# Lumina-Group/libzkp

Hardware: NVIDIA B200
Metric: groth16_bn254_proofs_per_sec_batched (higher is better)
Workload: dtype u256 (8x32-bit Montgomery limbs, integer)

## Files before the change

### libzkp_b200/csrc/engine.cu

```cuda
#include <cuda_runtime.h>
#include <atomic>
#include <cmath>
#include <cstdio>
#include <cstdlib>
#include <mutex>
#include <string>
#include <thread>
#include <type_traits>
#include <vector>

#include "common.h"
#include "host_util.h"
#include "kernels_prove.cuh"
#include "tables.h"
#include "large.h"
#include "setup.h"
#include "verify.h"

using namespace lzkp;
using namespace lzkp::eng;

static thread_local std::string g_err;
static std::mutex g_mu;
static int g_device = -1;
static std::vector<int> g_devices;
static thread_local int t_device = -1;
static uint64_t g_mimc_uploaded = 0;
static std::atomic<int> g_profile{0};

namespace lzkp {
namespace eng {
std::atomic<uint64_t> g_launches{0};
int fail(int code, const std::string &msg) {
    g_err = msg;
    return code;
}
int DBuf::alloc(size_t n) {
    release();
    if (n == 0) n = 16;
    cudaError_t e = cudaMalloc(&p, n);
    if (e != cudaSuccess) {
        p = nullptr;
        cudaGetLastError();
        return fail(LZKP_E_NOMEM, "cudaMalloc(" + std::to_string(n) + "): " + cudaGetErrorString(e));
    }
    bytes = n;
    return LZKP_OK;
}
void DBuf::release() {
    if (p) cudaFree(p);
    p = nullptr;
    bytes = 0;
}
int ensure_device() {
    std::lock_guard<std::mutex> lk(g_mu);
    if (g_device < 0) {
        int n = 0;
        cudaError_t e = cudaGetDeviceCount(&n);
        if (e != cudaSuccess || n == 0) {
            cudaGetLastError();
            return fail(LZKP_E_NO_DEVICE, "no CUDA device: this engine has no CPU fallback");
        }
        int dev = 0;
        if (const char *lr = getenv("LOCAL_RANK")) dev = atoi(lr) % n;
        g_device = dev;
    }
    const int dev = t_device >= 0 ? t_device : g_device;
    CUDA_TRY(cudaSetDevice(dev));
    if (!(g_mimc_uploaded >> (dev & 63) & 1)) {
        std::vector<Fr> c(110);
        for (uint32_t i = 0; i < 110; i++) c[i] = host::mimc_constant(i);
        CUDA_TRY(cudaMemcpyToSymbol(c_mimc, c.data(), sizeof(Fr) * 110));
        g_mimc_uploaded |= 1ull << (dev & 63);
    }
    return LZKP_OK;
}
int current_device() { return t_device >= 0 ? t_device : g_device; }
DeviceScope::DeviceScope(int dev) : prev(t_device) {
    t_device = dev;
    cudaSetDevice(dev);
}
DeviceScope::~DeviceScope() {
    t_device = prev;
    const int back = prev >= 0 ? prev : g_device;
    if (back >= 0) cudaSetDevice(back);
}
}
}


struct MsmPlan {
    DBuf table;
    DBuf unit_dig, unit_tbl;
    DBuf items[4];
    DBuf msm_items[4];
    uint32_t n_items[4] = {0, 0, 0, 0};
    uint32_t n_units = 0, n_rows = 0, n_msm = 0;
    std::vector<uint32_t> msm_unit_begin;
    std::vector<uint2> msm_items_host[4];
};
static const uint32_t kUnitsPerItem[4] = {8, 32, 128, 512};

struct HBuf {
    void *p = nullptr;
    size_t bytes = 0;
    int ensure(size_t n) {
        if (n <= bytes) return LZKP_OK;
        if (p) cudaFreeHost(p);
        p = nullptr;
        bytes = 0;
        cudaError_t err = cudaMallocHost(&p, n);
        if (err != cudaSuccess) { p = nullptr; cudaGetLastError(); return fail(LZKP_E_NOMEM, "cudaMallocHost failed"); }
        bytes = n;
        return LZKP_OK;
    }
    template <class T> T *as() const { return reinterpret_cast<T *>(p); }
    ~HBuf() { if (p) cudaFreeHost(p); }
};
struct Workspace {
    uint32_t chunk = 0;
    DBuf z, abc, tmp, h, dig, r, s, rs, part1, part2, res1, res2, proofs, status, a, b, commit, sets, setlen, env, envlen;
    HBuf h_proofs, h_status, h_commit, h_env, h_envlen;
    cudaEvent_t last_use = nullptr;
    ~Workspace() { if (last_use) cudaEventDestroy(last_use); }
};
static int ws_acquire(Workspace &ws, cudaStream_t st) {
    if (!ws.last_use) CUDA_TRY(cudaEventCreateWithFlags(&ws.last_use, cudaEventDisableTiming));
    else CUDA_TRY(cudaStreamWaitEvent(st, ws.last_use, 0));
    return LZKP_OK;
}
static int ws_release(Workspace &ws, cudaStream_t st) {
    CUDA_TRY(cudaEventRecord(ws.last_use, st));
    return LZKP_OK;
}

struct lzkp_pk {
    std::mutex mu;
    int device = 0;
    std::vector<lzkp_pk *> replicas;
    uint32_t n_vars = 0, n_inst = 0, n_wit = 0, n = 0, log_n = 0, m = 0;
    bool has_circuit = false;
    int kind = -1;
    uint32_t kind_param = 0;
    int c = 16;
    uint32_t W = 16, N = 32768;
    uint64_t table_bytes = 0;
    uint32_t max_chunk = 8192;
    uint32_t n_dig_rows = 0, nz = 0;
    MsmPlan g1, g2;
    MsmPlan g1_lat;
    uint32_t row_sz = 0, row_rz = 0;
    bool has_lat = false;
    ProofConsts consts;
    DBuf csr_rowptr[3], csr_col[3], csr_val[3];
    CsrDev csr[3];
    DBuf tw_fwd, tw_inv, coset_br, uncoset_br;
    NttTables ntt;
    Workspace ws[2];
    bool large = false;
    bool tiled_wm = false;
    MsmBases *L_a = nullptr, *L_b1 = nullptr, *L_b2 = nullptr, *L_l = nullptr, *L_h = nullptr;
    DBuf L_sa, L_sb, L_sl, L_sb1;
    cudaStream_t L_st[3] = {nullptr, nullptr, nullptr}, L_st_scale = nullptr;
    cudaEvent_t L_ev_in = nullptr, L_ev_done[3] = {nullptr, nullptr, nullptr}, L_ev_a = nullptr, L_ev_scale = nullptr;
    uint32_t shard_index = 0, shard_count = 1, map_ranks = 1;
    bool L_scaled = false;
    uint32_t L_lo[5] = {0, 0, 0, 0, 0}, L_cnt[5] = {0, 0, 0, 0, 0};
    cudaStream_t stream = nullptr, stream2 = nullptr;
    cudaEvent_t ev_fork = nullptr, ev_join[2] = {nullptr, nullptr};
    cudaStream_t chunk_stream(int i) const { return (i & 1) ? stream2 : stream; }
    struct Mark { int region; cudaEvent_t a, b; };
    std::vector<Mark> marks;
    double prof_ms[LZKP_PROFILE_REGIONS] = {0};
    uint64_t prof_count[LZKP_PROFILE_REGIONS] = {0};
    ~lzkp_pk() {
        for (lzkp_pk *r : replicas) { DeviceScope ds(r->device); delete r; }
        for (auto &m : marks) { cudaEventDestroy(m.a); cudaEventDestroy(m.b); }
        for (MsmBases *b : {L_a, L_b1, L_b2, L_l, L_h}) if (b) msm_bases_free(b);
        for (auto s_ : L_st) if (s_) cudaStreamDestroy(s_);
        if (L_ev_in) cudaEventDestroy(L_ev_in);
        if (L_ev_a) cudaEventDestroy(L_ev_a);
        if (L_ev_scale) cudaEventDestroy(L_ev_scale);
        if (L_st_scale) cudaStreamDestroy(L_st_scale);
        for (auto ev : L_ev_done) if (ev) cudaEventDestroy(ev);
        if (ev_fork) cudaEventDestroy(ev_fork);
        for (auto ev : ev_join) if (ev) cudaEventDestroy(ev);
        if (stream2) cudaStreamDestroy(stream2);
        if (stream) cudaStreamDestroy(stream);
    }
};

struct BaseRef { uint32_t dig_row, tbl_row; };
static int finish_plan(MsmPlan &pl, const std::vector<std::vector<BaseRef>> &msms, uint32_t W) {
    std::vector<uint32_t> ud, ut;
    pl.msm_unit_begin.clear();
    for (auto &ms : msms) {
        pl.msm_unit_begin.push_back((uint32_t)ud.size());
        for (auto &b : ms)
            for (uint32_t w = 0; w < W; w++) {
                ud.push_back(b.dig_row * W + w);
                ut.push_back(b.tbl_row * W + w);
            }
    }
    pl.msm_unit_begin.push_back((uint32_t)ud.size());
    pl.n_units = (uint32_t)ud.size();
    pl.n_msm = (uint32_t)msms.size();
    TRY(upload(pl.unit_dig, ud));
    TRY(upload(pl.unit_tbl, ut));
    for (int v = 0; v < 4; v++) {
        std::vector<uint2> items, mi;
        for (uint32_t q = 0; q < pl.n_msm; q++) {
            uint32_t first = (uint32_t)items.size();
            for (uint32_t u = pl.msm_unit_begin[q]; u < pl.msm_unit_begin[q + 1]; u += kUnitsPerItem[v])
                items.push_back(make_uint2(u, std::min(u + kUnitsPerItem[v], pl.msm_unit_begin[q + 1])));
            mi.push_back(make_uint2(first, (uint32_t)items.size()));
        }
        pl.n_items[v] = (uint32_t)items.size();
        pl.msm_items_host[v] = mi;
        TRY(upload(pl.items[v], items));
        TRY(upload(pl.msm_items[v], mi));
    }
    return LZKP_OK;
}

static inline uint32_t window_count(int c) { return (uint32_t)((255 + c - 1) / c); }

namespace {
struct Reader {
    const uint8_t *p, *end;
    bool take(size_t n, const uint8_t **out) {
        if ((size_t)(end - p) < n) return false;
        *out = p;
        p += n;
        return true;
    }
    bool g1(host::G1Canon &o) { const uint8_t *b; return take(64, &b) && host::read_g1(b, o); }
    bool g2(host::G2Canon &o) { const uint8_t *b; return take(128, &b) && host::read_g2(b, o); }
    bool vec_g1(std::vector<host::G1Canon> &v) {
        const uint8_t *b;
        if (!take(8, &b)) return false;
        uint64_t len;
        memcpy(&len, b, 8);
        if (len > (uint64_t)(end - p) / 64) return false;
        v.resize(len);
        for (auto &x : v) if (!g1(x)) return false;
        return true;
    }
    bool vec_g2(std::vector<host::G2Canon> &v) {
        const uint8_t *b;
        if (!take(8, &b)) return false;
        uint64_t len;
        memcpy(&len, b, 8);
        if (len > (uint64_t)(end - p) / 128) return false;
        v.resize(len);
        for (auto &x : v) if (!g2(x)) return false;
        return true;
    }
};
host::G1Canon neg_canon(const host::G1Canon &p) {
    host::G1Canon r = p;
    if (!host::is_inf(p)) {
        Fq m = Fq::modulus();
        sub8(r.y.l, m.l, p.y.l);
    }
    return r;
}
}

static int pk_load_impl(const uint8_t *bytes, size_t len, int validate, const lzkp_pk_options *opt, lzkp_pk *pk) {
    static_assert(sizeof(host::G1Canon) == sizeof(G1Affine) && sizeof(host::G2Canon) == sizeof(G2Affine), "layout");
    Reader rd{bytes, bytes + len};
    host::G1Canon alpha_g1, beta_g1, delta_g1;
    host::G2Canon beta_g2, gamma_g2, delta_g2;
    std::vector<host::G1Canon> gamma_abc, a_q, b1_q, h_q, l_q;
    std::vector<host::G2Canon> b2_q;
    bool ok = rd.g1(alpha_g1) && rd.g2(beta_g2) && rd.g2(gamma_g2) && rd.g2(delta_g2) && rd.vec_g1(gamma_abc) &&
              rd.g1(beta_g1) && rd.g1(delta_g1) && rd.vec_g1(a_q) && rd.vec_g1(b1_q) && rd.vec_g2(b2_q) &&
              rd.vec_g1(h_q) && rd.vec_g1(l_q);
    if (!ok || rd.p != rd.end) return fail(LZKP_E_INVALID, "proving key: malformed ark-serialize bytes");
    const uint32_t nv = (uint32_t)a_q.size();
    if (nv < 2 || b1_q.size() != nv || b2_q.size() != nv || l_q.size() >= nv || gamma_abc.size() + l_q.size() != nv)
        return fail(LZKP_E_INVALID, "proving key: inconsistent query lengths");
    const uint32_t n = (uint32_t)h_q.size() + 1;
    if (n < 2 || (n & (n - 1))) return fail(LZKP_E_INVALID, "proving key: h_query length + 1 is not a power of two");
    pk->n_vars = nv;
    pk->n_wit = (uint32_t)l_q.size();
    pk->n_inst = nv - pk->n_wit;
    pk->n = n;
    pk->log_n = 0;
    while ((1u << pk->log_n) < n) pk->log_n++;
    pk->nz = nv - 1;
    pk->n_dig_rows = pk->nz + 3 + (n - 1);
    const uint32_t ROW_R = pk->nz, ROW_S = pk->nz + 1, ROW_RS = pk->nz + 2, ROW_H = pk->nz + 3;

    {
        size_t free_b0 = 0, total_b0 = 0;
        CUDA_TRY(cudaMemGetInfo(&free_b0, &total_b0));
        const uint64_t budget0 = opt && opt->table_budget_bytes ? opt->table_budget_bytes : (uint64_t)(free_b0 * 0.6);
        const uint64_t rows1_max = 2ull * nv + pk->n_wit + n + 2, rows2_max = (uint64_t)nv + 1;
        const uint64_t min_table = (rows1_max * 64 + rows2_max * 128) * 32 * 128;
        pk->large = pk->log_n > 16 || min_table > budget0 || getenv("LZKP_FORCE_LARGE") != nullptr;
    }
    if (pk->large) {
        CUDA_TRY(cudaStreamCreate(&pk->stream));
    CUDA_TRY(cudaStreamCreate(&pk->stream2));
// ... 50 lines not shown
            pk->L_cnt[3] = 0;
        }
        double acc_w = 0;
        for (int q : {0, 1, 2, 4}) {
            auto first_at = [&](double w) -> uint64_t {
                if (w <= acc_w) return 0;
                return std::min<uint64_t>((uint64_t)std::ceil((w - acc_w) / wts[q]), sizes[q]);
            };
            uint64_t lo = first_at(cutz[me]), hi = me + 1 == G_ ? sizes[q] : first_at(cutz[me + 1]);
            pk->L_lo[q] = (uint32_t)lo;
            pk->L_cnt[q] = (uint32_t)(hi - lo);
            acc_w += (double)sizes[q] * wts[q];
        }
        auto load1 = [&](std::vector<host::G1Canon> v, size_t skip, const host::G1Canon *extra, int q, MsmBases **out) {
            v.erase(v.begin(), v.begin() + skip);
            if (extra) v.push_back(*extra);
            return msm_bases_load(1, reinterpret_cast<const uint8_t *>(v.data() + pk->L_lo[q]), pk->L_cnt[q], wb, 1, validate, out, 1);
        };
        host::G1Canon nd1 = neg_canon(delta_g1);
        TRY(load1(a_q, 1, &delta_g1, 0, &pk->L_a));
        TRY(load1(b1_q, 1, &delta_g1, 1, &pk->L_b1));
        TRY(load1(l_q, 0, &nd1, 2, &pk->L_l));
        TRY(load1(h_q, 0, nullptr, 3, &pk->L_h));
        {
            std::vector<host::G2Canon> v(b2_q.begin() + 1, b2_q.end());
            v.push_back(delta_g2);
            TRY(msm_bases_load(2, reinterpret_cast<const uint8_t *>(v.data() + pk->L_lo[4]), pk->L_cnt[4], wb, 1, validate, &pk->L_b2, 1));
        }
        {
            int prio_lo = 0, prio_hi = 0;
            CUDA_TRY(cudaDeviceGetStreamPriorityRange(&prio_lo, &prio_hi));
            const bool prio = !(getenv("LZKP_NO_STREAM_PRIORITY") && atoi(getenv("LZKP_NO_STREAM_PRIORITY")));
            for (int i = 0; i < 3; i++)
                CUDA_TRY(cudaStreamCreateWithPriority(&pk->L_st[i], cudaStreamNonBlocking, prio_lo));
            CUDA_TRY(cudaStreamCreateWithPriority(&pk->L_st_scale, cudaStreamNonBlocking, prio ? prio_hi : prio_lo));
        }
        CUDA_TRY(cudaEventCreateWithFlags(&pk->L_ev_in, cudaEventDisableTiming));
        CUDA_TRY(cudaEventCreateWithFlags(&pk->L_ev_a, cudaEventDisableTiming));
        CUDA_TRY(cudaEventCreateWithFlags(&pk->L_ev_scale, cudaEventDisableTiming));
        for (auto &ev : pk->L_ev_done) CUDA_TRY(cudaEventCreateWithFlags(&ev, cudaEventDisableTiming));
        pk->c = wb ? wb : 16;
        pk->W = (255 + pk->c - 1) / pk->c;
        pk->max_chunk = 1;
        pk->table_bytes = ((uint64_t)(a_q.size() + b1_q.size() + l_q.size() + 1 + h_q.size()) * 64 + (uint64_t)b2_q.size() * 128) * pk->W;
        std::vector<host::G1Canon> misc1 = {alpha_g1, beta_g1, a_q[0], b1_q[0]};
        std::vector<host::G2Canon> misc2 = {beta_g2, b2_q[0]};
        DBuf d_misc1, d_misc2, d_out1, d_out2;
        cudaStream_t st = pk->stream;
        TRY(upload(d_misc1, misc1)); TRY(upload(d_misc2, misc2));
        LAUNCH(k_fq_to_mont, 1, 128, 0, st, d_misc1.as<Fq>(), misc1.size() * 2);
        LAUNCH(k_fq_to_mont, 1, 128, 0, st, d_misc2.as<Fq>(), misc2.size() * 4);
        if (validate) {
            std::vector<host::G1Canon> v1 = gamma_abc;
            v1.push_back(alpha_g1); v1.push_back(beta_g1); v1.push_back(delta_g1); v1.push_back(a_q[0]); v1.push_back(b1_q[0]);
            std::vector<host::G2Canon> v2 = {beta_g2, gamma_g2, delta_g2, b2_q[0]};
            DBuf d_v1, d_v2, d_bad;
            TRY(upload(d_v1, v1)); TRY(upload(d_v2, v2)); TRY(d_bad.alloc(sizeof(int)));
            CUDA_TRY(cudaMemsetAsync(d_bad.p, 0, sizeof(int), st));
            LAUNCH(k_fq_to_mont, (unsigned)((v1.size() * 2 + 127) / 128), 128, 0, st, d_v1.as<Fq>(), v1.size() * 2);
            LAUNCH(k_fq_to_mont, 1, 128, 0, st, d_v2.as<Fq>(), v2.size() * 4);
            LAUNCH(k_check_g1, (unsigned)((v1.size() + 63) / 64), 64, 0, st, d_v1.as<G1Affine>(), (uint32_t)v1.size(), d_bad.as<int>());
            LAUNCH(k_check_g2, 1, 64, 0, st, d_v2.as<G2Affine>(), (uint32_t)v2.size(), d_bad.as<int>());
            int bad = 0;
            CUDA_TRY(cudaMemcpyAsync(&bad, d_bad.p, sizeof(int), cudaMemcpyDeviceToHost, st));
            CUDA_TRY(cudaStreamSynchronize(st));
            if (bad) return fail(LZKP_E_INVALID, "proving key: " + std::to_string(bad) + " point(s) off-curve or outside the subgroup");
        }
        TRY(d_out1.alloc(2 * sizeof(G1Affine))); TRY(d_out2.alloc(sizeof(G2Affine)));
        LAUNCH((k_affine_add<Fq>), 1, 1, 0, st, d_misc1.as<G1Affine>() + 0, d_misc1.as<G1Affine>() + 2, d_out1.as<G1Affine>() + 0, 0);
        LAUNCH((k_affine_add<Fq>), 1, 1, 0, st, d_misc1.as<G1Affine>() + 1, d_misc1.as<G1Affine>() + 3, d_out1.as<G1Affine>() + 1, 0);
        LAUNCH((k_affine_add<Fq2>), 1, 1, 0, st, d_misc2.as<G2Affine>() + 0, d_misc2.as<G2Affine>() + 1, d_out2.as<G2Affine>(), 0);
        G1Affine c1[2];
        G2Affine c2;
        CUDA_TRY(cudaMemcpyAsync(c1, d_out1.p, sizeof(c1), cudaMemcpyDeviceToHost, st));
        CUDA_TRY(cudaMemcpyAsync(&c2, d_out2.p, sizeof(c2), cudaMemcpyDeviceToHost, st));
        CUDA_TRY(cudaStreamSynchronize(st));
        pk->consts.a0 = c1[0]; pk->consts.b0 = c1[1]; pk->consts.b2 = c2;
        CUDA_TRY(cudaGetLastError());
        return LZKP_OK;
    }

    std::vector<host::G1Canon> rows1;
    std::vector<host::G2Canon> rows2;
    std::vector<std::vector<BaseRef>> msm1(4), msm2(1);
    auto add1 = [&](const host::G1Canon &p) { rows1.push_back(p); return (uint32_t)rows1.size() - 1; };
    for (uint32_t j = 1; j < nv; j++) if (!host::is_inf(a_q[j])) msm1[0].push_back({j - 1, add1(a_q[j])});
    for (uint32_t j = 1; j < nv; j++) if (!host::is_inf(b1_q[j])) msm1[1].push_back({j - 1, add1(b1_q[j])});
    for (uint32_t j = 0; j < pk->n_wit; j++) if (!host::is_inf(l_q[j])) msm1[2].push_back({pk->n_inst + j - 1, add1(l_q[j])});
    for (uint32_t i = 0; i + 1 < n; i++) if (!host::is_inf(h_q[i])) msm1[3].push_back({ROW_H + i, add1(h_q[i])});
    if (!host::is_inf(delta_g1)) {
        uint32_t rd1 = add1(delta_g1), rnd1 = add1(neg_canon(delta_g1));
        msm1[0].push_back({ROW_R, rd1});
        msm1[1].push_back({ROW_S, rd1});
        msm1[2].push_back({ROW_RS, rnd1});
    }
    std::vector<std::vector<BaseRef>> msm1_lat;
    {
        pk->row_sz = pk->n_dig_rows;
        pk->row_rz = pk->n_dig_rows + pk->nz;
        msm1_lat = msm1;
        msm1_lat.resize(6);
        for (auto &b : msm1[0]) if (b.dig_row < pk->nz) msm1_lat[4].push_back({pk->row_sz + b.dig_row, b.tbl_row});
        for (auto &b : msm1[1]) if (b.dig_row < pk->nz) msm1_lat[5].push_back({pk->row_rz + b.dig_row, b.tbl_row});
        auto mont = [](const host::G1Canon &c) { return G1Affine{Fq::from_canonical(c.x), Fq::from_canonical(c.y)}; };
        auto canon = [](const G1Affine &m) { host::G1Canon c; c.x = m.x.to_canonical(); c.y = m.y.to_canonical(); return c; };
        auto sum2 = [&](const host::G1Canon &u, const host::G1Canon &v) {
            G1XYZZ t = host::is_inf(u) ? G1XYZZ::inf() : G1XYZZ::from_affine(mont(u));
            if (!host::is_inf(v)) t.madd(mont(v));
            return t.is_inf() ? host::G1Canon{Fq::zero(), Fq::zero()} : canon(t.to_affine());
        };
        const host::G1Canon a0c = sum2(alpha_g1, a_q[0]), b0c = sum2(beta_g1, b1_q[0]), d2c = sum2(delta_g1, delta_g1);
        if (!host::is_inf(a0c)) msm1_lat[4].push_back({ROW_S, add1(a0c)});
        if (!host::is_inf(b0c)) msm1_lat[5].push_back({ROW_R, add1(b0c)});
        if (!host::is_inf(d2c)) msm1_lat[5].push_back({ROW_RS, add1(d2c)});
        pk->n_dig_rows += 2 * pk->nz;
        pk->has_lat = true;
    }
    for (uint32_t j = 1; j < nv; j++)
        if (!host::is_inf(b2_q[j])) { rows2.push_back(b2_q[j]); msm2[0].push_back({j - 1, (uint32_t)rows2.size() - 1}); }
    if (!host::is_inf(delta_g2)) { rows2.push_back(delta_g2); msm2[0].push_back({ROW_S, (uint32_t)rows2.size() - 1}); }
    pk->g1.n_rows = (uint32_t)rows1.size();
    pk->g2.n_rows = (uint32_t)rows2.size();

    size_t free_b = 0, total_b = 0;
    CUDA_TRY(cudaMemGetInfo(&free_b, &total_b));
    uint64_t budget = opt && opt->table_budget_bytes ? opt->table_budget_bytes : (uint64_t)(free_b * 0.6);
    int c = opt && opt->window_bits ? opt->window_bits : 0;
    if (const char *e = getenv("LZKP_WINDOW_BITS")) if (!c) c = atoi(e);
    auto bytes_for = [&](int cc) {
        uint64_t W = window_count(cc), N = 1ull << (cc - 1);
        return (rows1.size() * 64ull + rows2.size() * 128ull) * W * N;
    };
    if (c == 0) {
        c = 16;
        while (c > 8 && bytes_for(c) > budget) c--;
    }
    if (c < 8 || c > 17) return fail(LZKP_E_INVALID, "window_bits must be in [8,17]");
    if (bytes_for(c) > free_b) return fail(LZKP_E_NOMEM, "window tables do not fit in device memory");
    pk->c = c;
    pk->W = window_count(c);
    pk->N = 1u << (c - 1);
    pk->table_bytes = bytes_for(c);
    pk->max_chunk = opt && opt->max_chunk ? opt->max_chunk : 8192;
    if (pk->max_chunk > 32768) pk->max_chunk = 32768;

    CUDA_TRY(cudaStreamCreate(&pk->stream));
    CUDA_TRY(cudaStreamCreate(&pk->stream2));
    CUDA_TRY(cudaEventCreateWithFlags(&pk->ev_fork, cudaEventDisableTiming));
    for (auto &ev : pk->ev_join) CUDA_TRY(cudaEventCreateWithFlags(&ev, cudaEventDisableTiming));
    CUDA_TRY(cudaStreamCreateWithFlags(&pk->L_st[0], cudaStreamNonBlocking));
    CUDA_TRY(cudaEventCreateWithFlags(&pk->L_ev_in, cudaEventDisableTiming));
    CUDA_TRY(cudaEventCreateWithFlags(&pk->L_ev_done[0], cudaEventDisableTiming));
    cudaStream_t st = pk->stream;

    std::vector<host::G1Canon> misc1 = {alpha_g1, beta_g1, delta_g1, a_q[0], b1_q[0]};
    std::vector<host::G2Canon> misc2 = {beta_g2, gamma_g2, delta_g2, b2_q[0]};
    DBuf d_rows1, d_rows2, d_misc1, d_misc2, d_out1, d_out2;
    TRY(upload(d_rows1, rows1)); TRY(upload(d_rows2, rows2)); TRY(upload(d_misc1, misc1)); TRY(upload(d_misc2, misc2));
    auto to_mont = [&](DBuf &b, size_t n_fq) {
        if (n_fq) LAUNCH(k_fq_to_mont, (unsigned)((n_fq + 127) / 128), 128, 0, st, b.as<Fq>(), n_fq);
    };
    to_mont(d_rows1, rows1.size() * 2); to_mont(d_rows2, rows2.size() * 4);
    to_mont(d_misc1, misc1.size() * 2); to_mont(d_misc2, misc2.size() * 4);
    if (validate) {
        std::vector<host::G1Canon> all1 = gamma_abc;
        std::vector<host::G2Canon> all2;
        DBuf d_all1, d_bad;
        TRY(upload(d_all1, all1));
        to_mont(d_all1, all1.size() * 2);
        TRY(d_bad.alloc(sizeof(int)));
        CUDA_TRY(cudaMemsetAsync(d_bad.p, 0, sizeof(int), st));
        auto chk1 = [&](DBuf &b, size_t cnt) {
            if (cnt) LAUNCH(k_check_g1, (unsigned)((cnt + 63) / 64), 64, 0, st, b.as<G1Affine>(), (uint32_t)cnt, d_bad.as<int>());
        };
        auto chk2 = [&](DBuf &b, size_t cnt) {
            if (cnt) LAUNCH(k_check_g2, (unsigned)((cnt + 63) / 64), 64, 0, st, b.as<G2Affine>(), (uint32_t)cnt, d_bad.as<int>());
        };
        chk1(d_rows1, rows1.size()); chk1(d_misc1, misc1.size()); chk1(d_all1, all1.size());
        chk2(d_rows2, rows2.size()); chk2(d_misc2, misc2.size());
        int bad = 0;
        CUDA_TRY(cudaMemcpyAsync(&bad, d_bad.p, sizeof(int), cudaMemcpyDeviceToHost, st));
        CUDA_TRY(cudaStreamSynchronize(st));
        if (bad) return fail(LZKP_E_INVALID, "proving key: " + std::to_string(bad) + " point(s) off-curve or outside the subgroup");
    }
    TRY(d_out1.alloc(2 * sizeof(G1Affine))); TRY(d_out2.alloc(sizeof(G2Affine)));
    LAUNCH((k_affine_add<Fq>), 1, 1, 0, st, d_misc1.as<G1Affine>() + 0, d_misc1.as<G1Affine>() + 3, d_out1.as<G1Affine>() + 0, 0);
    LAUNCH((k_affine_add<Fq>), 1, 1, 0, st, d_misc1.as<G1Affine>() + 1, d_misc1.as<G1Affine>() + 4, d_out1.as<G1Affine>() + 1, 0);
    LAUNCH((k_affine_add<Fq2>), 1, 1, 0, st, d_misc2.as<G2Affine>() + 0, d_misc2.as<G2Affine>() + 3, d_out2.as<G2Affine>(), 0);
    G1Affine c1[2];
    G2Affine c2;
    CUDA_TRY(cudaMemcpyAsync(c1, d_out1.p, sizeof(c1), cudaMemcpyDeviceToHost, st));
    CUDA_TRY(cudaMemcpyAsync(&c2, d_out2.p, sizeof(c2), cudaMemcpyDeviceToHost, st));
    CUDA_TRY(cudaStreamSynchronize(st));
    pk->consts.a0 = c1[0]; pk->consts.b0 = c1[1]; pk->consts.b2 = c2;

    TRY(pk->g1.table.alloc((size_t)rows1.size() * pk->W * pk->N * sizeof(G1Affine)));
    TRY(pk->g2.table.alloc((size_t)rows2.size() * pk->W * pk->N * sizeof(G2Affine)));
    if (!rows1.empty())
        TRY(build_table_g1(d_rows1.p, (uint32_t)rows1.size(), c, pk->W, pk->N, pk->g1.table.p, st));
    if (!rows2.empty())
        TRY(build_table_g2(d_rows2.p, (uint32_t)rows2.size(), c, pk->W, pk->N, pk->g2.table.p, st));
    TRY(finish_plan(pk->g1, msm1, pk->W));
    TRY(finish_plan(pk->g1_lat, msm1_lat, pk->W));
    TRY(finish_plan(pk->g2, msm2, pk->W));
    {
        const uint64_t per_proof = (uint64_t)nv * 32 + 7ull * n * 32 + (uint64_t)pk->n_dig_rows * pk->W * (c > 16 ? 4 : 2) +
                                   (uint64_t)pk->g1.n_items[2] * sizeof(G1XYZZ) + (uint64_t)pk->g2.n_items[1] * sizeof(G2XYZZ) +
                                   4 * sizeof(G1XYZZ) + sizeof(G2XYZZ) + 1024;
        size_t free_now = 0, total_now = 0;
        CUDA_TRY(cudaMemGetInfo(&free_now, &total_now));
        uint64_t fit = (uint64_t)(free_now * 0.4) / (2 * per_proof);
        fit = std::max<uint64_t>(32, fit / 32 * 32);
        if (pk->max_chunk > fit) pk->max_chunk = (uint32_t)fit;
    }
    CUDA_TRY(cudaGetLastError());
    return LZKP_OK;
}

static int circuit_install(lzkp_pk *pk, uint32_t m, uint32_t n_inst, uint32_t n_wit, const uint32_t *const rowptr[3],
                           const uint32_t *const col[3], const uint8_t *const val[3]) {
    if (n_inst != pk->n_inst || n_wit != pk->n_wit) return fail(LZKP_E_INVALID, "circuit shape does not match the proving key");
    uint64_t need = (uint64_t)m + n_inst;
    uint32_t n = 1;
    while (n < need) n <<= 1;
    if (n != pk->n) return fail(LZKP_E_INVALID, "circuit domain size does not match the proving key's h_query");
    pk->tiled_wm = pk->large || pk->log_n > 12;
    cudaStream_t st = pk->stream;
    for (int k = 0; k < 3; k++) {
        uint32_t nnz = rowptr[k][m];
        for (uint32_t i = 0; i < nnz; i++) if (col[k][i] >= pk->n_vars) return fail(LZKP_E_INVALID, "matrix column out of range");
        TRY(pk->csr_rowptr[k].alloc(sizeof(uint32_t) * (m + 1)));
        TRY(pk->csr_col[k].alloc(sizeof(uint32_t) * nnz));
        TRY(pk->csr_val[k].alloc(sizeof(Fr) * (size_t)nnz));
        CUDA_TRY(cudaMemcpy(pk->csr_rowptr[k].p, rowptr[k], sizeof(uint32_t) * (m + 1), cudaMemcpyHostToDevice));
        if (nnz) {
            CUDA_TRY(cudaMemcpy(pk->csr_col[k].p, col[k], sizeof(uint32_t) * nnz, cudaMemcpyHostToDevice));
            CUDA_TRY(cudaMemcpy(pk->csr_val[k].p, val[k], 32 * (size_t)nnz, cudaMemcpyHostToDevice));
            LAUNCH(k_to_r2_form, (nnz + 127) / 128, 128, 0, st, pk->csr_val[k].as<Fr>(), nnz);
        }
        pk->csr[k] = CsrDev{pk->csr_rowptr[k].as<uint32_t>(), pk->csr_col[k].as<uint32_t>(), pk->csr_val[k].as<Fr>()};
    }
    pk->m = m;
    Fr w, wi, g, gi;
    for (int i = 0; i < 8; i++) { w.l[i] = FrParams::ROOT28(i); wi.l[i] = FrParams::ROOT28_INV(i); g.l[i] = FrParams::GEN(i); gi.l[i] = FrParams::GEN_INV(i); }
    for (uint32_t i = pk->log_n; i < 28; i++) { w = w.sqr(); wi = wi.sqr(); }
    Fr ninv = host::fr_from_u64(n).inverse();
    Fr gn = g;
    for (uint32_t i = 0; i < pk->log_n; i++) gn = gn.sqr();
    Fr zinv = (gn - Fr::one()).inverse();
    if (pk->tiled_wm) {
        pk->ntt = NttTables{nullptr, nullptr, nullptr, nullptr, nullptr, ninv, zinv};
        CUDA_TRY(cudaStreamSynchronize(st));
        CUDA_TRY(cudaGetLastError());
        pk->has_circuit = true;
        return LZKP_OK;
    }
    TRY(pk->tw_fwd.alloc(sizeof(Fr) * (n / 2))); TRY(pk->tw_inv.alloc(sizeof(Fr) * (n / 2)));
    TRY(pk->coset_br.alloc(sizeof(Fr) * n)); TRY(pk->uncoset_br.alloc(sizeof(Fr) * n));
    LAUNCH(k_pow_table, (n / 2 + 127) / 128, 128, 0, st, pk->tw_fwd.as<Fr>(), w, Fr::one(), n / 2, 0u);
    LAUNCH(k_pow_table, (n / 2 + 127) / 128, 128, 0, st, pk->tw_inv.as<Fr>(), wi, Fr::one(), n / 2, 0u);
    LAUNCH(k_pow_table, (n + 127) / 128, 128, 0, st, pk->coset_br.as<Fr>(), g, ninv, n, pk->log_n);
    LAUNCH(k_pow_table, (n + 127) / 128, 128, 0, st, pk->uncoset_br.as<Fr>(), gi, ninv.to_canonical(), n, pk->log_n);
    pk->ntt = NttTables{pk->tw_fwd.as<Fr>(), pk->tw_inv.as<Fr>(), pk->coset_br.as<Fr>(), pk->uncoset_br.as<Fr>(), nullptr, ninv, zinv};
    size_t smem = (size_t)32 * n;
    if (smem > 48 * 1024) {
        CUDA_TRY(cudaFuncSetAttribute(k_ntt_icoset, cudaFuncAttributeMaxDynamicSharedMemorySize, (int)smem));
        CUDA_TRY(cudaFuncSetAttribute(k_ntt_final, cudaFuncAttributeMaxDynamicSharedMemorySize, (int)smem));
    }
    CUDA_TRY(cudaStreamSynchronize(st));
    CUDA_TRY(cudaGetLastError());
    pk->has_circuit = true;
    return LZKP_OK;
}

static inline int item_variant(uint32_t P) {
    return P > small_batch_limit() ? (P >= 256 ? 2 : 1) : 0;
}
static inline int fit_variant(const MsmPlan &pl, int v) {
    while (v < 3 && pl.n_items[v] > 65535u) v++;
    return v;
}
static inline uint32_t latency_limit() {
    static const uint32_t v = getenv("LZKP_LATENCY_BATCH") ? (uint32_t)atoi(getenv("LZKP_LATENCY_BATCH")) : 384u;
    return v;
// ... 988 lines not shown
```

### libzkp_b200/csrc/kernels_prove.cuh

```cuda
#pragma once
#include "dev_util.cuh"

namespace lzkp {

__global__ void k_pow_table(Fr *out, Fr base, Fr scale, uint32_t count, uint32_t log_rev) {
    uint32_t k = blockIdx.x * blockDim.x + threadIdx.x;
    if (k >= count) return;
    uint32_t e = log_rev ? bitrev(k, log_rev) : k;
    Fr acc = Fr::one(), b = base;
    while (e) {
        if (e & 1u) acc = acc * b;
        b = b.sqr();
        e >>= 1;
    }
    st_vec(out + k, acc * scale);
}
__global__ void k_to_r2_form(Fr *v, uint32_t count) {
    uint32_t k = blockIdx.x * blockDim.x + threadIdx.x;
    if (k >= count) return;
    Fr r3;
#pragma unroll
    for (int i = 0; i < 8; i++) r3.l[i] = FrParams::R3(i);
    st_vec(v + k, ld_vec(v + k) * r3);
}
// ... 234 lines not shown
__global__ void k_fr_to_canonical(Fr *v, size_t n) {
    size_t i = (size_t)blockIdx.x * blockDim.x + threadIdx.x;
    if (i >= n) return;
    st_vec(v + i, ld_vec(v + i).to_canonical());
}
__global__ void k_check_canonical(const Fr *v, uint32_t count, int32_t *status) {
    uint32_t i = blockIdx.x * blockDim.x + threadIdx.x;
    if (i >= count) return;
    if (!fr_is_canonical(ld_vec(v + i))) status[0] = 1;
}

template <class DigT>
__global__ void __launch_bounds__(128) k_digits(const Fr *scalars, uint32_t stride, uint32_t first, DigT *dig,
                                                uint32_t row0, uint32_t P, uint32_t c, uint32_t W, int32_t *status,
                                                uint32_t count) {
    uint32_t p = blockIdx.x * blockDim.x + threadIdx.x;
    if (p >= P) return;
    for (uint32_t j = blockIdx.y; j < count; j += gridDim.y) {
        Fr s = ld_vec(scalars + (size_t)p * stride + first + j);
        if (!fr_is_canonical(s)) {
            status[p] = 1;
            s = Fr::zero();
        }
        uint32_t v[10];
        recode_offset(s, c, W, v);
        const size_t base = ((size_t)(row0 + j) * W) * P + p;
        for (uint32_t w = 0; w < W; w++) dig[base + (size_t)w * P] = (DigT)recoded_digit(v, c, w);
    }
}
template <class DigT>
__global__ void __launch_bounds__(128) k_digits_scaled(const Fr *scalars, uint32_t stride, uint32_t first, const Fr *mult,
                                                       DigT *dig, uint32_t row0, uint32_t P, uint32_t c, uint32_t W,
                                                       uint32_t count) {
    uint32_t p = blockIdx.x * blockDim.x + threadIdx.x;
    if (p >= P) return;
    Fr m = ld_vec(mult + p);
    if (!fr_is_canonical(m)) m = Fr::zero();
    const Fr mr2 = m * Fr::r2();
    for (uint32_t j = blockIdx.y; j < count; j += gridDim.y) {
        Fr z = ld_vec(scalars + (size_t)p * stride + first + j);
        if (!fr_is_canonical(z)) z = Fr::zero();
        const Fr s = z * mr2;
        uint32_t v[10];
        recode_offset(s, c, W, v);
        const size_t base = ((size_t)(row0 + j) * W) * P + p;
        for (uint32_t w = 0; w < W; w++) dig[base + (size_t)w * P] = (DigT)recoded_digit(v, c, w);
    }
}
__global__ void k_fr_mul_canonical(const Fr *r, const Fr *s, Fr *rs, uint32_t P) {
    uint32_t p = blockIdx.x * blockDim.x + threadIdx.x;
    if (p >= P) return;
    st_vec(rs + p, (ld_vec(r + p) * ld_vec(s + p)) * Fr::r2());
}

struct ProofConsts {
    G1Affine a0;
    G1Affine b0;
    G2Affine b2;
};
__device__ __forceinline__ G1XYZZ glv_half(const G1XYZZ &P, const Fr &k, int half) {
    GlvSplit sp = glv_split(k);
    if (!sp.ok) return half == 0 ? scalar_mul(P, k) : G1XYZZ::inf();
    G1XYZZ Q = P;
    if (half == 1) {
        Fq beta;
#pragma unroll
        for (int i = 0; i < 8; i++) beta.l[i] = FqParams::BETA(i);
        Q.x = Q.x * beta;
    }
    if (half == 0 ? sp.neg1 : sp.neg2) Q.y = Q.y.neg();
    return half == 0 ? scalar_mul_u128(Q, sp.k1) : scalar_mul_u128(Q, sp.k2);
}
__global__ void __launch_bounds__(128) k_assemble(const G1XYZZ *g1, const G2XYZZ *g2, ProofConsts K, const Fr *r,
                                                  const Fr *s, uint32_t P, uint8_t *proofs) {
    __shared__ uint4 sm_raw[3 * 32 * sizeof(G1XYZZ) / 16];
    G1XYZZ *sm = reinterpret_cast<G1XYZZ *>(sm_raw);
    const uint32_t role = threadIdx.x >> 5, lane = threadIdx.x & 31, p = blockIdx.x * 32 + lane;
    const bool live = p < P;
    uint8_t *out = proofs + (size_t)p * 256;
    G1XYZZ acc = G1XYZZ::inf(), A = G1XYZZ::inf();
    if (live) {
        if (role <= 1) {
            A = ld_vec(g1 + p);
            A.madd_cold(K.a0);
            if (role == 0) acc = glv_half(A, ld_vec(s + p), 0);
            else st_vec(sm + lane, glv_half(A, ld_vec(s + p), 1));
        } else {
            G1XYZZ B1 = ld_vec(g1 + (size_t)P + p);
            B1.madd_cold(K.b0);
            st_vec(sm + (role - 1) * 32 + lane, glv_half(B1, ld_vec(r + p), role - 2));
        }
    }
    __syncthreads();
    if (!live) return;
    if (role == 0) {
        acc.add_cold(ld_vec(sm + lane));
        acc.add_cold(ld_vec(sm + 32 + lane));
        acc.add_cold(ld_vec(sm + 64 + lane));
        acc.add_cold(ld_vec(g1 + 2 * (size_t)P + p));
        acc.add_cold(ld_vec(g1 + 3 * (size_t)P + p));
        write_g1(out + 192, acc.to_affine());
    } else if (role == 1) {
        write_g1(out, A.to_affine());
    } else if (role == 2) {
        G2XYZZ B2 = ld_vec(g2 + p);
        B2.madd_cold(K.b2);
        write_g2(out + 64, B2.to_affine());
    }
}

__global__ void __launch_bounds__(128) k_scale_a(G1XYZZ *g1, ProofConsts K, const Fr *r, const Fr *s, int with_consts) {
    __shared__ uint4 sm_raw[3 * sizeof(G1XYZZ) / 16];
    G1XYZZ *sm = reinterpret_cast<G1XYZZ *>(sm_raw);
    const uint32_t role = threadIdx.x >> 5, lane = threadIdx.x & 31;
    G1XYZZ acc = G1XYZZ::inf();
    if (lane == 0 && (role <= 1 || with_consts)) {
        G1XYZZ X = role <= 1 ? ld_vec(g1) : G1XYZZ::from_affine(K.b0);
        if (role <= 1 && with_consts) X.madd_cold(K.a0);
        acc = glv_half(X, ld_vec(role <= 1 ? s : r), role & 1);
    }
    if (lane == 0 && role) st_vec(sm + (role - 1), acc);
    __syncthreads();
    if (threadIdx.x == 0) {
        acc.add_cold(ld_vec(sm));
        acc.add_cold(ld_vec(sm + 1));
        acc.add_cold(ld_vec(sm + 2));
        st_vec(g1 + 4, acc);
    }
}
__global__ void k_scalars_times(const Fr *z, const Fr *k, Fr *out, uint32_t count) {
    const uint32_t i = blockIdx.x * blockDim.x + threadIdx.x;
    if (i >= count) return;
    st_vec(out + i, (ld_vec(z + i) * ld_vec(k)) * Fr::r2());
}
__global__ void k_add_slot(G1XYZZ *g1, int dst, int src) {
    G1XYZZ a = ld_vec(g1 + dst);
    a.add_cold(ld_vec(g1 + src));
    st_vec(g1 + dst, a);
}

__global__ void __launch_bounds__(96) k_assemble_sums(const G1XYZZ *g1, const G2XYZZ *g2, ProofConsts K, uint32_t P,
                                                      uint8_t *proofs, int q0, int q1) {
    const uint32_t role = threadIdx.x >> 5, lane = threadIdx.x & 31, p = blockIdx.x * 32 + lane;
    if (p >= P) return;
    uint8_t *out = proofs + (size_t)p * 256;
    if (role == 0) {
        G1XYZZ acc = ld_vec(g1 + (size_t)q0 * P + p);
        if (q1 >= 0) acc.add_cold(ld_vec(g1 + (size_t)q1 * P + p));
        acc.add_cold(ld_vec(g1 + 2 * (size_t)P + p));
        acc.add_cold(ld_vec(g1 + 3 * (size_t)P + p));
        write_g1(out + 192, acc.to_affine());
    } else if (role == 1) {
        G1XYZZ A = ld_vec(g1 + p);
        A.madd_cold(K.a0);
        write_g1(out, A.to_affine());
    } else {
        G2XYZZ B2 = ld_vec(g2 + p);
        B2.madd_cold(K.b2);
        write_g2(out + 64, B2.to_affine());
    }
}

__global__ void __launch_bounds__(128) k_envelope(const uint8_t *proofs, const uint8_t *commit, const int32_t *status,
                                                  const uint64_t *sets, const uint32_t *set_len, uint32_t set_stride,
                                                  uint32_t scheme, uint32_t P, uint8_t *out, uint32_t out_stride,
                                                  uint32_t *out_len) {
    const uint32_t p = (blockIdx.x * blockDim.x + threadIdx.x) >> 5, lane = threadIdx.x & 31;
    if (p >= P) return;
    uint8_t *o = out + (size_t)p * out_stride;
    if (status[p] != 0) {
        if (lane == 0) out_len[p] = 0;
// ... 62 lines not shown
```

### libzkp_b200/csrc/msm_batch.cu

```cuda
#include <cstdlib>
#include "tables.h"
#include "dev_util.cuh"

#ifndef LZKP_G2_MINB
#define LZKP_G2_MINB 6
#endif
#ifndef LZKP_G1_MINB
#define LZKP_G1_MINB 4
#endif
#define LZKP_G2_MINB_SEL(F) (sizeof(F) == sizeof(::lzkp::Fq) ? LZKP_G1_MINB : LZKP_G2_MINB)
namespace lzkp {

template <class F, int BLOCK, class DigT>
__global__ void __launch_bounds__(BLOCK, LZKP_G2_MINB_SEL(F)) k_msm_batch(const Affine<F> *__restrict__ table, uint32_t N,
                                                     const uint32_t *__restrict__ unit_dig,
                                                     const uint32_t *__restrict__ unit_tbl,
                                                     const uint2 *__restrict__ items, const DigT *__restrict__ dig,
                                                     uint32_t P, XYZZ<F> *__restrict__ partial) {
    const uint32_t p = blockIdx.x * BLOCK + threadIdx.x, item = blockIdx.y;
    if (p >= P) return;
    const uint2 range = items[item];
    XYZZ<F> acc = XYZZ<F>::inf();
    int d = dig[(size_t)__ldg(unit_dig + range.x) * P + p];
    Affine<F> pt = Affine<F>::inf();
    if (d) pt = gather_point(table, N, __ldg(unit_tbl + range.x), d);
    for (uint32_t u = range.x; u < range.y; u++) {
        int dn = 0;
        Affine<F> ptn = Affine<F>::inf();
        if (u + 1 < range.y) {
            dn = dig[(size_t)__ldg(unit_dig + u + 1) * P + p];
            if (dn) ptn = gather_point(table, N, __ldg(unit_tbl + u + 1), dn);
        }
        if (d) acc.madd(pt);
        d = dn;
        pt = ptn;
    }
    st_vec(partial + (size_t)item * P + p, acc);
}
template <class F>
__global__ void __launch_bounds__(128) k_msm_reduce1(XYZZ<F> *partial, const uint2 *msm_items, uint32_t P, uint32_t G) {
    uint32_t p = blockIdx.x * blockDim.x + threadIdx.x, q = blockIdx.y, g = blockIdx.z;
    if (p >= P) return;
    uint2 r = msm_items[q];
    if (r.x + g >= r.y) return;
    XYZZ<F> acc = ld_vec(partial + (size_t)(r.x + g) * P + p);
    for (uint32_t it = r.x + g + G; it < r.y; it += G) acc.add_cold(ld_vec(partial + (size_t)it * P + p));
    st_vec(partial + (size_t)(r.x + g) * P + p, acc);
}
template <class F>
__global__ void __launch_bounds__(128) k_msm_reduce(const XYZZ<F> *partial, const uint2 *msm_items, uint32_t P,
                                                    uint32_t G, XYZZ<F> *out) {
    uint32_t p = blockIdx.x * blockDim.x + threadIdx.x, q = blockIdx.y;
    if (p >= P) return;
    uint2 r = msm_items[q];
    uint32_t end = min(r.y, r.x + G);
    XYZZ<F> acc = XYZZ<F>::inf();
    for (uint32_t it = r.x; it < end; it++) acc.add_cold(ld_vec(partial + (size_t)it * P + p));
    st_vec(out + (size_t)q * P + p, acc);
}

template <class F>
__global__ void __launch_bounds__(128) k_msm_fold(XYZZ<F> *partial, const uint2 *msm_items, uint32_t P, uint32_t half,
                                                  XYZZ<F> *out) {
    uint32_t p = blockIdx.x * blockDim.x + threadIdx.x, q = blockIdx.y, g = blockIdx.z;
    if (p >= P) return;
    const uint2 r = msm_items[q];
    const uint32_t live = min(r.y - r.x, 2 * half);
    if (g >= live) {
        if (half == 1 && g == 0) st_vec(out + (size_t)q * P + p, XYZZ<F>::inf());
        return;
    }
    XYZZ<F> acc = ld_vec(partial + (size_t)(r.x + g) * P + p);
    if (g + half < live) acc.add_cold(ld_vec(partial + (size_t)(r.x + g + half) * P + p));
    if (half == 1) st_vec(out + (size_t)q * P + p, acc);
    else st_vec(partial + (size_t)(r.x + g) * P + p, acc);
}

template <class F, int T>
__global__ void __launch_bounds__(T) k_msm_reduce_tree(const XYZZ<F> *__restrict__ partial, const uint2 *__restrict__ msm_items,
                                                       uint32_t P, XYZZ<F> *__restrict__ out) {
    __shared__ uint4 raw[T * sizeof(XYZZ<F>) / 16];
    XYZZ<F> *sm = reinterpret_cast<XYZZ<F> *>(raw);
    const uint32_t p = blockIdx.x, q = blockIdx.y, t = threadIdx.x;
    const uint2 r = msm_items[q];
    XYZZ<F> acc = XYZZ<F>::inf();
    for (uint32_t it = r.x + t; it < r.y; it += T) acc.add_cold(ld_vec(partial + (size_t)it * P + p));
    st_vec(sm + t, acc);
    __syncthreads();
    for (uint32_t s = T / 2; s > 0; s >>= 1) {
        if (t < s) {
            XYZZ<F> a = ld_vec(sm + t);
            a.add_cold(ld_vec(sm + t + s));
            st_vec(sm + t, a);
        }
        __syncthreads();
    }
    if (t == 0) st_vec(out + (size_t)q * P + p, ld_vec(sm));
}

}

namespace lzkp {
namespace eng {
uint32_t small_batch_limit() {
    static const uint32_t v = [] {
        const char *e = getenv("LZKP_SMALL_BATCH");
        return e ? (uint32_t)atoi(e) : 512u;
    }();
    return v;
}

void batch_msm_g1_items(const BatchMsmArgs &a, uint32_t item0, uint32_t count, cudaStream_t st) {
    if (!count) return;
    if (a.P <= small_batch_limit()) {
        if (a.dig_bytes == 2)
            LAUNCH((k_msm_batch<Fq, 32, int16_t>), dim3((a.P + 31) / 32, count), 32, 0, st, (const G1Affine *)a.table, a.N, a.unit_dig, a.unit_tbl,
                   (const uint2 *)a.items + item0, (const int16_t *)a.dig, a.P, (G1XYZZ *)a.partial + (size_t)item0 * a.P);
        else
            LAUNCH((k_msm_batch<Fq, 32, int32_t>), dim3((a.P + 31) / 32, count), 32, 0, st, (const G1Affine *)a.table, a.N, a.unit_dig, a.unit_tbl,
                   (const uint2 *)a.items + item0, (const int32_t *)a.dig, a.P, (G1XYZZ *)a.partial + (size_t)item0 * a.P);
        return;
    }
    if (a.dig_bytes == 2)
        LAUNCH((k_msm_batch<Fq, 128, int16_t>), dim3((a.P + 127) / 128, count), 128, 0, st, (const G1Affine *)a.table, a.N, a.unit_dig,
               a.unit_tbl, (const uint2 *)a.items + item0, (const int16_t *)a.dig, a.P, (G1XYZZ *)a.partial + (size_t)item0 * a.P);
    else
        LAUNCH((k_msm_batch<Fq, 128, int32_t>), dim3((a.P + 127) / 128, count), 128, 0, st, (const G1Affine *)a.table, a.N, a.unit_dig,
               a.unit_tbl, (const uint2 *)a.items + item0, (const int32_t *)a.dig, a.P, (G1XYZZ *)a.partial + (size_t)item0 * a.P);
}
constexpr uint32_t kReduceFan = 8;
void batch_msm_g1_reduce(const BatchMsmArgs &a, cudaStream_t st) {
    if (a.P <= small_batch_limit()) {
        LAUNCH((k_msm_reduce_tree<Fq, 128>), dim3(a.P, a.n_msm), 128, 0, st, (const G1XYZZ *)a.partial, (const uint2 *)a.msm_items,
               a.P, (G1XYZZ *)a.out);
        return;
    }
    LAUNCH((k_msm_reduce1<Fq>), dim3((a.P + 127) / 128, a.n_msm, kReduceFan), 128, 0, st, (G1XYZZ *)a.partial,
           (const uint2 *)a.msm_items, a.P, kReduceFan);
    for (uint32_t half = kReduceFan / 2; half >= 1; half >>= 1)
        LAUNCH((k_msm_fold<Fq>), dim3((a.P + 127) / 128, a.n_msm, half), 128, 0, st, (G1XYZZ *)a.partial,
               (const uint2 *)a.msm_items, a.P, half, (G1XYZZ *)a.out);
}
void batch_msm_g1(const BatchMsmArgs &a, cudaStream_t st) {
    batch_msm_g1_items(a, 0, a.n_items, st);
    batch_msm_g1_reduce(a, st);
}
void batch_msm_g2(const BatchMsmArgs &a, cudaStream_t st) {
    if (a.P <= small_batch_limit()) {
        if (a.dig_bytes == 2)
            LAUNCH((k_msm_batch<Fq2, 32, int16_t>), dim3((a.P + 31) / 32, a.n_items), 32, 0, st, (const G2Affine *)a.table, a.N, a.unit_dig,
                   a.unit_tbl, (const uint2 *)a.items, (const int16_t *)a.dig, a.P, (G2XYZZ *)a.partial);
        else
            LAUNCH((k_msm_batch<Fq2, 32, int32_t>), dim3((a.P + 31) / 32, a.n_items), 32, 0, st, (const G2Affine *)a.table, a.N, a.unit_dig,
                   a.unit_tbl, (const uint2 *)a.items, (const int32_t *)a.dig, a.P, (G2XYZZ *)a.partial);
        LAUNCH((k_msm_reduce_tree<Fq2, 128>), dim3(a.P, a.n_msm), 128, 0, st, (const G2XYZZ *)a.partial, (const uint2 *)a.msm_items,
               a.P, (G2XYZZ *)a.out);
        return;
    }
    if (a.dig_bytes == 2)
        LAUNCH((k_msm_batch<Fq2, 64, int16_t>), dim3((a.P + 63) / 64, a.n_items), 64, 0, st, (const G2Affine *)a.table, a.N,
               a.unit_dig, a.unit_tbl, (const uint2 *)a.items, (const int16_t *)a.dig, a.P, (G2XYZZ *)a.partial);
    else
        LAUNCH((k_msm_batch<Fq2, 64, int32_t>), dim3((a.P + 63) / 64, a.n_items), 64, 0, st, (const G2Affine *)a.table, a.N,
               a.unit_dig, a.unit_tbl, (const uint2 *)a.items, (const int32_t *)a.dig, a.P, (G2XYZZ *)a.partial);
    LAUNCH((k_msm_reduce1<Fq2>), dim3((a.P + 127) / 128, a.n_msm, 2 * kReduceFan), 128, 0, st, (G2XYZZ *)a.partial,
           (const uint2 *)a.msm_items, a.P, 2 * kReduceFan);
    for (uint32_t half = kReduceFan; half >= 1; half >>= 1)
        LAUNCH((k_msm_fold<Fq2>), dim3((a.P + 127) / 128, a.n_msm, half), 128, 0, st, (G2XYZZ *)a.partial,
               (const uint2 *)a.msm_items, a.P, half, (G2XYZZ *)a.out);
}

}
}
```

### libzkp_b200/csrc/tables.h

```cpp
#pragma once
#include "common.h"

namespace lzkp {
namespace eng {

int build_table_g1(const void *d_bases, uint32_t rows, int c, uint32_t W, uint32_t N, void *d_table, cudaStream_t st);
int build_table_g2(const void *d_bases, uint32_t rows, int c, uint32_t W, uint32_t N, void *d_table, cudaStream_t st);

struct BatchMsmArgs {
    const void *table;
    uint32_t N;
    const uint32_t *unit_dig, *unit_tbl;
    const void *items;
    uint32_t n_items;
    const void *msm_items;
    uint32_t n_msm;
    const void *dig;
    uint32_t dig_bytes;
    uint32_t P;
    void *partial;
    void *out;
};
void batch_msm_g1(const BatchMsmArgs &a, cudaStream_t st);
void batch_msm_g1_items(const BatchMsmArgs &a, uint32_t item0, uint32_t count, cudaStream_t st);
void batch_msm_g1_reduce(const BatchMsmArgs &a, cudaStream_t st);
void batch_msm_g2(const BatchMsmArgs &a, cudaStream_t st);
uint32_t small_batch_limit();

}
}
```

Before: 171,500.

## Merge shared A/B1 query bases into one MSM and fit item length to occupancy

Wire terms whose A and B1 G1 query points are identical go into a new fifth MSM, so each such base is handled once instead of twice. The prove kernel adds that shared partial sum into both the A and B1 accumulators. The latency plan is rebuilt from the merged lists. Separately, the third item-length variant is now picked at setup by a cost model that uses the device's resident block count, replacing a fixed 128, to cut tail-wave imbalance. Risks are the extra point add per proof, reliance on duplicated points being common, and correctness of the plan reshuffle.

```diff
diff --git a/libzkp_b200/csrc/engine.cu b/libzkp_b200/csrc/engine.cu
--- a/libzkp_b200/csrc/engine.cu
+++ b/libzkp_b200/csrc/engine.cu
@@ -95,11 +95,11 @@
     DBuf items[4];
     DBuf msm_items[4];
     uint32_t n_items[4] = {0, 0, 0, 0};
+    uint32_t item_len[4] = {8, 32, 128, 512};
     uint32_t n_units = 0, n_rows = 0, n_msm = 0;
     std::vector<uint32_t> msm_unit_begin;
     std::vector<uint2> msm_items_host[4];
 };
-static const uint32_t kUnitsPerItem[4] = {8, 32, 128, 512};
 
 struct HBuf {
     void *p = nullptr;
@@ -211,8 +211,8 @@
         std::vector<uint2> items, mi;
         for (uint32_t q = 0; q < pl.n_msm; q++) {
             uint32_t first = (uint32_t)items.size();
-            for (uint32_t u = pl.msm_unit_begin[q]; u < pl.msm_unit_begin[q + 1]; u += kUnitsPerItem[v])
-                items.push_back(make_uint2(u, std::min(u + kUnitsPerItem[v], pl.msm_unit_begin[q + 1])));
+            for (uint32_t u = pl.msm_unit_begin[q]; u < pl.msm_unit_begin[q + 1]; u += pl.item_len[v])
+                items.push_back(make_uint2(u, std::min(u + pl.item_len[v], pl.msm_unit_begin[q + 1])));
             mi.push_back(make_uint2(first, (uint32_t)items.size()));
         }
         pl.n_items[v] = (uint32_t)items.size();
@@ -221,6 +221,18 @@
         TRY(upload(pl.msm_items[v], mi));
     }
     return LZKP_OK;
+}
+
+static uint32_t fit_item_len(const std::vector<std::vector<BaseRef>> &msms, uint32_t W, uint32_t resident) {
+    uint32_t best = 128;
+    uint64_t best_cost = UINT64_MAX;
+    for (uint32_t len = 96; len <= 192; len++) {
+        uint64_t items = 0, cost = 0;
+        for (auto &ms : msms) items += ((uint64_t)ms.size() * W + len - 1) / len;
+        for (uint64_t gx : {8u, 16u, 32u, 64u}) cost += (gx * items + resident - 1) / resident * len * (64 / gx);
+        if (cost < best_cost) { best_cost = cost; best = len; }
+    }
+    return best;
 }
 
 static inline uint32_t window_count(int c) { return (uint32_t)((255 + c - 1) / c); }
@@ -437,10 +449,22 @@
 
     std::vector<host::G1Canon> rows1;
     std::vector<host::G2Canon> rows2;
-    std::vector<std::vector<BaseRef>> msm1(4), msm2(1);
+    std::vector<std::vector<BaseRef>> msm1(5), msm2(1);
+    std::vector<BaseRef> a_all, b1_all;
     auto add1 = [&](const host::G1Canon &p) { rows1.push_back(p); return (uint32_t)rows1.size() - 1; };
-    for (uint32_t j = 1; j < nv; j++) if (!host::is_inf(a_q[j])) msm1[0].push_back({j - 1, add1(a_q[j])});
-    for (uint32_t j = 1; j < nv; j++) if (!host::is_inf(b1_q[j])) msm1[1].push_back({j - 1, add1(b1_q[j])});
+    auto same_point = [](const host::G1Canon &u, const host::G1Canon &v) {
+        return memcmp(&u.x, &v.x, sizeof(Fq)) == 0 && memcmp(&u.y, &v.y, sizeof(Fq)) == 0;
+    };
+    for (uint32_t j = 1; j < nv; j++) {
+        const bool has_a = !host::is_inf(a_q[j]), has_b = !host::is_inf(b1_q[j]);
+        if (has_a && has_b && same_point(a_q[j], b1_q[j])) {
+            const BaseRef ref{j - 1, add1(a_q[j])};
+            msm1[4].push_back(ref); a_all.push_back(ref); b1_all.push_back(ref);
+            continue;
+        }
+        if (has_a) { msm1[0].push_back({j - 1, add1(a_q[j])}); a_all.push_back(msm1[0].back()); }
+        if (has_b) { msm1[1].push_back({j - 1, add1(b1_q[j])}); b1_all.push_back(msm1[1].back()); }
+    }
     for (uint32_t j = 0; j < pk->n_wit; j++) if (!host::is_inf(l_q[j])) msm1[2].push_back({pk->n_inst + j - 1, add1(l_q[j])});
     for (uint32_t i = 0; i + 1 < n; i++) if (!host::is_inf(h_q[i])) msm1[3].push_back({ROW_H + i, add1(h_q[i])});
     if (!host::is_inf(delta_g1)) {
@@ -448,15 +472,17 @@
         msm1[0].push_back({ROW_R, rd1});
         msm1[1].push_back({ROW_S, rd1});
         msm1[2].push_back({ROW_RS, rnd1});
-    }
-    std::vector<std::vector<BaseRef>> msm1_lat;
+        a_all.push_back({ROW_R, rd1});
+    }
+    std::vector<std::vector<BaseRef>> msm1_lat(6);
     {
         pk->row_sz = pk->n_dig_rows;
         pk->row_rz = pk->n_dig_rows + pk->nz;
-        msm1_lat = msm1;
-        msm1_lat.resize(6);
-        for (auto &b : msm1[0]) if (b.dig_row < pk->nz) msm1_lat[4].push_back({pk->row_sz + b.dig_row, b.tbl_row});
-        for (auto &b : msm1[1]) if (b.dig_row < pk->nz) msm1_lat[5].push_back({pk->row_rz + b.dig_row, b.tbl_row});
+        msm1_lat[0] = a_all;
+        msm1_lat[2] = msm1[2];
+        msm1_lat[3] = msm1[3];
+        for (auto &b : a_all) if (b.dig_row < pk->nz) msm1_lat[4].push_back({pk->row_sz + b.dig_row, b.tbl_row});
+        for (auto &b : b1_all) msm1_lat[5].push_back({pk->row_rz + b.dig_row, b.tbl_row});
         auto mont = [](const host::G1Canon &c) { return G1Affine{Fq::from_canonical(c.x), Fq::from_canonical(c.y)}; };
         auto canon = [](const G1Affine &m) { host::G1Canon c; c.x = m.x.to_canonical(); c.y = m.y.to_canonical(); return c; };
         auto sum2 = [&](const host::G1Canon &u, const host::G1Canon &v) {
@@ -555,6 +581,11 @@
         TRY(build_table_g1(d_rows1.p, (uint32_t)rows1.size(), c, pk->W, pk->N, pk->g1.table.p, st));
     if (!rows2.empty())
         TRY(build_table_g2(d_rows2.p, (uint32_t)rows2.size(), c, pk->W, pk->N, pk->g2.table.p, st));
+    {
+        uint32_t resident = 0;
+        TRY(batch_msm_g1_resident(c > 16 ? 4 : 2, &resident));
+        pk->g1.item_len[2] = fit_item_len(msm1, pk->W, resident);
+    }
     TRY(finish_plan(pk->g1, msm1, pk->W));
     TRY(finish_plan(pk->g1_lat, msm1_lat, pk->W));
     TRY(finish_plan(pk->g2, msm2, pk->W));
diff --git a/libzkp_b200/csrc/kernels_prove.cuh b/libzkp_b200/csrc/kernels_prove.cuh
--- a/libzkp_b200/csrc/kernels_prove.cuh
+++ b/libzkp_b200/csrc/kernels_prove.cuh
@@ -340,11 +340,13 @@
     if (live) {
         if (role <= 1) {
             A = ld_vec(g1 + p);
+            A.add_cold(ld_vec(g1 + 4 * (size_t)P + p));
             A.madd_cold(K.a0);
             if (role == 0) acc = glv_half(A, ld_vec(s + p), 0);
             else st_vec(sm + lane, glv_half(A, ld_vec(s + p), 1));
         } else {
             G1XYZZ B1 = ld_vec(g1 + (size_t)P + p);
+            B1.add_cold(ld_vec(g1 + 4 * (size_t)P + p));
             B1.madd_cold(K.b0);
             st_vec(sm + (role - 1) * 32 + lane, glv_half(B1, ld_vec(r + p), role - 2));
         }
diff --git a/libzkp_b200/csrc/msm_batch.cu b/libzkp_b200/csrc/msm_batch.cu
--- a/libzkp_b200/csrc/msm_batch.cu
+++ b/libzkp_b200/csrc/msm_batch.cu
@@ -1,3 +1,4 @@
+#include <algorithm>
 #include <cstdlib>
 #include "tables.h"
 #include "dev_util.cuh"
@@ -110,6 +111,16 @@
     return v;
 }
 
+int batch_msm_g1_resident(uint32_t dig_bytes, uint32_t *out) {
+    int dev = 0, sms = 0, per_sm = 0;
+    CUDA_TRY(cudaGetDevice(&dev));
+    CUDA_TRY(cudaDeviceGetAttribute(&sms, cudaDevAttrMultiProcessorCount, dev));
+    if (dig_bytes == 2) CUDA_TRY(cudaOccupancyMaxActiveBlocksPerMultiprocessor(&per_sm, k_msm_batch<Fq, 128, int16_t>, 128, 0));
+    else CUDA_TRY(cudaOccupancyMaxActiveBlocksPerMultiprocessor(&per_sm, k_msm_batch<Fq, 128, int32_t>, 128, 0));
+    *out = (uint32_t)std::max(1, sms * per_sm);
+    return LZKP_OK;
+}
+
 void batch_msm_g1_items(const BatchMsmArgs &a, uint32_t item0, uint32_t count, cudaStream_t st) {
     if (!count) return;
     if (a.P <= small_batch_limit()) {
diff --git a/libzkp_b200/csrc/tables.h b/libzkp_b200/csrc/tables.h
--- a/libzkp_b200/csrc/tables.h
+++ b/libzkp_b200/csrc/tables.h
@@ -25,6 +25,7 @@
 void batch_msm_g1_items(const BatchMsmArgs &a, uint32_t item0, uint32_t count, cudaStream_t st);
 void batch_msm_g1_reduce(const BatchMsmArgs &a, cudaStream_t st);
 void batch_msm_g2(const BatchMsmArgs &a, cudaStream_t st);
+int batch_msm_g1_resident(uint32_t dig_bytes, uint32_t *out);
 uint32_t small_batch_limit();
 
 }
```

Result: faster. 178,500, median of 6 (+4.1%).
